# Harvard-AI-and-Robotics-Lab/FairFedMed

Measured on AMD Instinct MI355X. Metric: images/sec per client-round, ViT-B/16 FairLoRA r=8, bs=32 224^2, higher is better.
Workload: dtype bf16; 1 GPU; configs[1]: 1-client ViT-B/16 FairLoRA rank=8 G=3, bs=32 synthetic 224x224x3, fwd+bwd+SGD per step; global_batch=32, clients=1, trainable_elems=741952, loss_finite=1, launch=replay, rccl_ranks=1

## Files before the change

### fairfedmed_amd/_lib.py

```python
from __future__ import annotations

import ctypes as C
import os
from typing import Optional

import torch

_HERE = os.path.dirname(os.path.abspath(__file__))
LIB_PATH = os.environ.get("FFM_LIB_PATH") or os.path.join(_HERE, "csrc", "libffm_hip.so")

F32, BF16, F32_X3, F16 = 0, 1, 2, 3
F32_X3_W16 = 4
EPI_BIAS, EPI_LORA, EPI_LORA_KR, EPI_RESIDUAL, EPI_GELU, EPI_DGELU, EPI_RANKOP = 1, 2, 4, 8, 16, 32, 64
EPI_ROWSTATS, EPI_LNIN, EPI_LGRAD, EPI_BNBWD = 128, 256, 512, 1024
EPI_LNB_STAT, EPI_LNB_APPLY = 2048, 4096
EPI_GELU_ONLY = 8192
ABI_VERSION = 14
FILTERS = {"bilinear": 0, "bicubic": 1}

_vp, _i32, _i64, _f32 = C.c_void_p, C.c_int32, C.c_int64, C.c_float


class GemmArgs(C.Structure):
    _fields_ = [
# ... 79 lines not shown
    "ffm_ot_head_fwd": [_vp] * 10 + [_i32] * 6 + [_f32, _f32, _i32, _f32, _i32, _vp],
    "ffm_ot_head_bwd": [_vp] * 8 + [_i32] * 6 + [_vp],
    "ffm_expand_u8": [_vp, _vp, _i32, _i32, _i32, _i32, _vp],
    "ffm_resize_u8": [_vp, _vp, _vp, _vp, _vp, _i32, _i32, _i32, _i32, _i32, _vp],
    "ffm_augment_taps": [_i32, _i32, _i32],
    "ffm_augment_boxes": [_vp, _vp, _i32, _i64, _i32, _i32, _i32, _vp, _vp, _vp],
    "ffm_crop_resize_u8": [_vp, _vp, _vp, _vp, _i32, _i32, _i32, _i32, _i32, _i32, _vp],
    "ffm_scale_check": [_vp, _f32, _i64, _vp, _vp],
    "ffm_attention_fwd": [_vp, _vp, _vp, _i32, _i32, _i32, _i32, _i32, _vp],
    "ffm_attention_bwd": [_vp, _vp, _vp, _vp, _vp, _vp, _i32, _i32, _i32, _i32, _i32, _vp],
    "ffm_attention_bwd_lnstat_ok": [_i32, _i32, _i32],
    "ffm_attention_route": [_i32, _i32, _i32],
    "ffm_attention_bwd_lnstat": [_vp, _vp, _vp, _vp, _vp, _vp, _vp, _vp, _vp, _i32, _i32, _i32, _i32, _i32, _vp],
    "ffm_lora_down": [_vp, _i32, _vp, _i32, _vp, _vp, _i32, _i32, _i32, _i32, _i32, _f32, _f32, _vp, _vp, _vp, _vp,
                      _i32, _vp],
    "ffm_lora_down_blocks": [_i32, _i32, _i32, _i32],
    "ffm_lora_down_blocks_max": [_i32, _i32, _i32, _i32],
    "ffm_lora_grad_partial": [_vp, _i32, _vp, _i32, _i32, _i32, _vp, _i32, _vp],
    "ffm_lora_grad_partial_ln": [_vp, _i32, _vp, _vp, _vp, _vp, _vp, _i32, _i32, _i32, _vp, _i32, _vp],
    "ffm_lora_grad_splits": [_i32],
    "ffm_reduce_partials": [_vp, _i32, _i32, _vp, _i32, _i32, _i32, _vp],
    "ffm_reduce_partials_multi": [_vp, _i32, _i32, _vp],
    "ffm_head_fwd": [_vp, _vp, _vp, _vp, _vp, _vp, _i32, _i32, _i32, _i32, _i32, _vp],
    "ffm_ce_loss": [_vp, _vp, _vp, _vp, _vp, _vp, _vp, _i32, _i32, _i32, _vp],
    "ffm_ce_fair_loss": [_vp] * 10 + [_i32, _i32, _i32, _i32, _f32, _i32, _vp],
    "ffm_head_bwd": [_vp, _vp, _vp, _vp, _vp, _vp, _vp, _vp, _i32, _i32, _i32, _i32, _i32, _vp],
    "ffm_text_embed": [_vp, _vp, _vp, _i32, _vp, _vp, _i32, _i32, _i32, _i32, _i32, _vp],
    "ffm_text_tail_fwd": [_vp] * 10 + [_i32] * 4 + [_vp],
    "ffm_text_tail_bwd": [_vp] * 11 + [_i32] * 5 + [_vp],
    "ffm_text_ctx_grad": [_vp, _vp, _i32, _i32, _i32, _i32, _i32, _vp],
    "ffm_sgd_momentum": [_vp, _vp, _vp, _i64, _f32, _f32, _f32, _i32, _vp],
    "ffm_sgd_momentum_n": [_vp, _vp, _vp, _i64, _f32, _f32, _f32, _i32, _i32, _vp],
    "ffm_sgd_momentum_dev": [_vp, _vp, _vp, _i64, _vp, _i32, _vp, _vp],
    "ffm_loss_scale": [_vp, _i64, _vp, _vp],
    "ffm_unscale_check": [_vp, _i64, _vp, _vp],
    "ffm_sgd_momentum_gated": [_vp, _vp, _vp, _i64, _f32, _f32, _f32, _i32, _i32, _vp, _vp],
    "ffm_optim_state_rows": [_i32],
    "ffm_optim_step": [_vp, _vp, _vp, _i64, _i32, _vp, _i32, _vp, _vp],
    "ffm_optim_step_dev": [_vp, _vp, _vp, _i64, _i32, _vp, _i32, _vp, _vp],
    "ffm_scale_by": [_vp, _vp, _vp, _i64, _vp],
    "ffm_scale_acc": [_vp, _vp, _vp, _i64, _vp],
    "ffm_fedavg_finish": [_vp, _vp, _vp, _i64, _vp, _i32, _i32, _i32, _i32, _f32, _vp],
    "ffm_dp_norm_ws_bytes": [_i64],
    "ffm_dp_norm": [_vp, _vp, _i64, _vp, _vp],
    "ffm_dp_privatise": [_vp, _vp, _vp, _vp, _i64, _vp, _f32, _f32, _i64, _i32, _i32, _i32, _vp, _vp],
    "ffm_dp_noise": [_vp, _i64, _f32, _i64, _i32, _i32, _vp],
# ... 57 lines not shown
```

### fairfedmed_amd/csrc/head.hip

```cpp
#include "common.h"

namespace {

constexpr int HD_MAXV = 4;
constexpr int HD_MAXC = 8;

constexpr int HD_NW = 16;

template <typename T>
__global__ __launch_bounds__(64 * HD_NW) void head_fwd_kernel(const T* __restrict__ f, const float* __restrict__ tbar,
                                                       const float* __restrict__ logit_scale,
                                                       float* __restrict__ fbar, float* __restrict__ rnorm,
                                                       float* __restrict__ logits, int L, int D, int n_cls) {
    __shared__ float red[HD_NW / 2][4 * 64 * HD_MAXV];
    const int b = blockIdx.x, lane = threadIdx.x & 63, wave = threadIdx.x >> 6;
    const int nchunk = D >> 2;
    f32x4 acc[HD_MAXV];
#pragma unroll
    for (int i = 0; i < HD_MAXV; ++i) acc[i] = (f32x4){0.f, 0.f, 0.f, 0.f};
    for (int l = 1 + wave; l < L; l += HD_NW) {
        const T* fr = f + ((size_t)b * L + l) * D;
        f32x4 v[HD_MAXV];
        float ss = 0.f;
#pragma unroll
// ... 35 lines not shown
            if (c < nchunk) {
#pragma unroll
                for (int e = 0; e < 4; ++e) red[wave][c * 4 + e] += acc[i][e];
            }
        }
    }
    __syncthreads();
    const float inv = 1.0f / (float)(L - 1);
    for (int d = threadIdx.x; d < D; d += 64 * HD_NW) {
        float s = 0.f;
#pragma unroll
        for (int w = 0; w < HD_NW / 2; ++w) s += red[w][d];
        s *= inv;
        red[0][d] = s;
        fbar[(size_t)b * D + d] = s;
    }
    __syncthreads();
    const float scale = expf(logit_scale[0]);
    for (int c = wave; c < n_cls; c += HD_NW) {
        float s = 0.f;
        for (int d = lane; d < D; d += 64) s += red[0][d] * tbar[(size_t)c * D + d];
        s = wave_sum(s);
        if (lane == 0) logits[(size_t)b * n_cls + c] = scale * s;
    }
}

__global__ __launch_bounds__(256) void ce_loss_kernel(const float* __restrict__ logits_img,
                                                      const int64_t* __restrict__ label, float* __restrict__ logits,
                                                      float* __restrict__ prob, float* __restrict__ loss,
                                                      float* __restrict__ dlogits_img, int32_t* __restrict__ finite,
                                                      int nb, int S, int n_cls) {
    __shared__ float part[256];
    float my = 0.f;
    for (int b = threadIdx.x; b < nb; b += 256) {
        float lg[HD_MAXC];
        float mx = -INFINITY;
        for (int c = 0; c < n_cls; ++c) {
            float s = 0.f;
            for (int k = 0; k < S; ++k) s += logits_img[((size_t)b * S + k) * n_cls + c];
            lg[c] = s / (float)S;
            logits[(size_t)b * n_cls + c] = lg[c];
            mx = fmaxf(mx, lg[c]);
        }
        float se = 0.f;
        for (int c = 0; c < n_cls; ++c) se += expf(lg[c] - mx);
        const float lse = mx + logf(se);
// ... 209 lines not shown
            fb[u] = fbar[(size_t)(b + u) * D + d];
        }
#pragma unroll
        for (int u = 0; u < 8; ++u) s += dl[u] * fb[u];
    }
    for (; b < B; ++b) s += dlogits[(size_t)b * n_cls + c] * fbar[(size_t)b * D + d];
    dtbar[i] = s * expf(logit_scale[0]);
}

}

extern "C" int ffm_head_fwd(const void* f, const float* tbar, const float* logit_scale, float* fbar, float* rnorm,
                            float* logits_img, int B, int L, int D, int n_cls, int dtype, void* stream) {
    if (!f || !tbar || !logit_scale || !fbar || !rnorm || !logits_img) return FFM_EINVAL;
    if (B <= 0 || L <= 1 || D <= 0 || (D & 3) || D > 4 * 64 * HD_MAXV || n_cls <= 0 || n_cls > HD_MAXC) return FFM_EINVAL;
    hipStream_t s = (hipStream_t)stream;
    return ffm_by_storage(dtype, [&](auto tag) {
        typedef typename decltype(tag)::type T;
        hipLaunchKernelGGL((head_fwd_kernel<T>), dim3(B), dim3(64 * HD_NW), 0, s, (const T*)f, tbar, logit_scale, fbar, rnorm,
                           logits_img, L, D, n_cls);
        FFM_CHECK_LAUNCH();
        return FFM_OK;
    });
}

extern "C" int ffm_ce_loss(const float* logits_img, const int64_t* label, float* logits, float* prob, float* loss,
                           float* dlogits_img, int32_t* finite_flag, int nb, int S, int n_cls, void* stream) {
    if (!logits_img || !label || !logits || !prob || !loss || !dlogits_img) return FFM_EINVAL;
    if (nb <= 0 || S <= 0 || n_cls <= 0 || n_cls > HD_MAXC) return FFM_EINVAL;
    hipLaunchKernelGGL(ce_loss_kernel, dim3(1), dim3(256), 0, (hipStream_t)stream, logits_img, label, logits, prob,
                       loss, dlogits_img, finite_flag, nb, S, n_cls);
    FFM_CHECK_LAUNCH();
    return FFM_OK;
}

extern "C" int ffm_ce_fair_loss(const float* logits_img, const int64_t* label, const int32_t* attr, float* logits,
                                float* prob, float* loss, float* terms, float* gstat, float* dlogits_img,
                                int32_t* finite_flag, int nb, int S, int n_cls, int G, float lambda, int with_grad,
                                void* stream) {
    if (!logits_img || !label || !attr || !logits || !prob || !loss || !terms || !dlogits_img) return FFM_EINVAL;
    if (nb <= 0 || S <= 0 || n_cls <= 0 || n_cls > HD_MAXC || G <= 0 || G > FFM_MAX_GROUPS) return FFM_EINVAL;
    hipLaunchKernelGGL(ce_fair_loss_kernel, dim3(1), dim3(256), 0, (hipStream_t)stream, logits_img, label, attr, logits,
                       prob, loss, terms, gstat, dlogits_img, finite_flag, nb, S, n_cls, G, lambda, with_grad ? 1 : 0);
    FFM_CHECK_LAUNCH();
    return FFM_OK;
}
// ... 21 lines not shown
```

### fairfedmed_amd/csrc/lora.hip

```cpp
#include "common.h"

namespace {

constexpr int LD_WAVES = 8;
constexpr int LD_LDS_BUDGET = 64 * 1024;

template <int V>
__device__ __forceinline__ void reduce_scatter64(float (&vals)[V], int lane) {
#pragma unroll
    for (int n = V, o = 32; o >= 1; n >>= 1, o >>= 1) {
        const bool up = (lane & o) != 0;
#pragma unroll
        for (int i = 0; i < n / 2; ++i) {
            const float a = vals[i], b = vals[i + n / 2];
            const float keep = up ? b : a, send = up ? a : b;
            vals[i] = keep + __shfl_xor(send, o, 64);
        }
    }
}

template <typename T, int RP>
__global__ __launch_bounds__(LD_WAVES * 64) void lora_down_kernel(
    const T* __restrict__ x, int ldx, const float* __restrict__ P, int layout_rk, const float* __restrict__ S,
    const int32_t* __restrict__ attr, int M, int K, int r, int G, int rows_per_sample, float scaling,
// ... 120 lines not shown
        float sbv = 0.f;
        for (int g = 0; g < G; ++g) sbv += group_mix_w(attr, sample, g, G, lambda_group) * S[g * rs + j0 + oj];
        if (t_out) t_out[(size_t)orow * rs + j0 + oj] = tval;
        if (ts_out) ts_out[(size_t)orow * rs + j0 + oj] = scaling * tval * sbv;
    }
    if (t_fwd && ds_part) {
        if (kq == 0)
            Vs[(rg * RSUB + lane / RP) * RP + oj] = writer ? scaling * t_fwd[(size_t)orow * rs + j0 + oj] * tval : 0.f;
        __syncthreads();
        if (tid < G * r) {
            const int g = tid / r, j = tid % r;
            float s = 0.f;
            for (int rr = 0; rr < rows_blk; ++rr) {
                const int grow = blockIdx.x * rows_blk + rr;
                if (grow < M) s += group_mix_w(attr, grow / rows_per_sample, g, G, lambda_group) * Vs[rr * RP + j];
            }
            ds_part[((size_t)blockIdx.x * G + g) * rs + j0 + j] = s;
        }
    }
}

constexpr int LDM_ROWS = 16, LDM_WAVES = 4, LDM_U = 4;

__global__ __launch_bounds__(LDM_WAVES * 64) void lora_down_mfma_kernel(
    const bf16_t* __restrict__ x, int ldx, const float* __restrict__ P, const float* __restrict__ S,
    const int32_t* __restrict__ attr, int M, int K, int r, int G, int rows_per_sample, float scaling, float lambda_group,
    float* __restrict__ t_out, float* __restrict__ ts_out, const float* __restrict__ t_fwd, float* __restrict__ ds_part) {
    __shared__ f32x4 red[LDM_WAVES][64];
    __shared__ float dsum[(FFM_MAX_GROUPS + 2) * 16];
    const int tid = threadIdx.x, lane = tid & 63, wave = tid >> 6;
    const int col = lane & 15, kgp = lane >> 4;
    const int row0 = blockIdx.x * LDM_ROWS;
    int arow = row0 + col;
    arow = arow < M ? arow : M - 1;
    const int ksl = K / LDM_WAVES;
    const bf16_t* xa = x + (size_t)arow * ldx + wave * ksl + kgp * 8;
    const float* pb = P + (size_t)(col < r ? col : 0) * K + wave * ksl + kgp * 8;
    const bool bok = col < r;
    f32x4 acc = {0.f, 0.f, 0.f, 0.f};
    const int steps = ksl >> 5;
    for (int s0 = 0; s0 < steps; s0 += LDM_U) {
        bf16x8 av[LDM_U];
        f32x4 b0[LDM_U], b1[LDM_U];
#pragma unroll
        for (int u = 0; u < LDM_U; ++u) {
            const int st = s0 + u < steps ? s0 + u : steps - 1;
            av[u] = *reinterpret_cast<const bf16x8*>(xa + st * 32);
            b0[u] = *reinterpret_cast<const f32x4*>(pb + st * 32);
            b1[u] = *reinterpret_cast<const f32x4*>(pb + st * 32 + 4);
        }
#pragma unroll
        for (int u = 0; u < LDM_U; ++u) {
            if (s0 + u >= steps) break;
            bf16x8 bv;
#pragma unroll
            for (int e = 0; e < 4; ++e) {
                bv[e] = bok ? (bf16_t)b0[u][e] : (bf16_t)0.f;
                bv[4 + e] = bok ? (bf16_t)b1[u][e] : (bf16_t)0.f;
            }
            acc = __builtin_amdgcn_mfma_f32_16x16x32_bf16(bv, av[u], acc, 0, 0, 0);
        }
    }
    red[wave][lane] = acc;
    __syncthreads();
    if (wave != 0) return;
    f32x4 t4 = red[0][lane];
#pragma unroll
    for (int w = 1; w < LDM_WAVES; ++w) {
        const f32x4 o = red[w][lane];
#pragma unroll
        for (int e = 0; e < 4; ++e) t4[e] += o[e];
    }
    const int grow = row0 + col;
    const bool rok = grow < M;
    const int sample = (rok ? grow : M - 1) / rows_per_sample;
    const int ga = attr ? group_id(attr[sample], G) : -1;
    const float w_own = lambda_group, w_oth = (1.0f - lambda_group) / (float)(G > 1 ? G - 1 : 1), w_uni = 1.0f / (float)G;
    const bool do_ds = t_fwd && ds_part;
    float wv[4];
#pragma unroll
    for (int e = 0; e < 4; ++e) {
        const int j = 4 * kgp + e;
        wv[e] = 0.f;
        if (j < r && rok) {
            float sb = 0.f;
            for (int g = 0; g < G; ++g) sb += (ga < 0 ? w_uni : (ga == g ? w_own : w_oth)) * S[g * r + j];
            if (t_out) t_out[(size_t)grow * r + j] = t4[e];
            if (ts_out) ts_out[(size_t)grow * r + j] = scaling * t4[e] * sb;
            if (do_ds) wv[e] = scaling * t_fwd[(size_t)grow * r + j] * t4[e];
        }
    }
    if (!do_ds) return;
    float d_all[4], d_uni[4];
#pragma unroll
    for (int e = 0; e < 4; ++e) {
        d_all[e] = ga < 0 ? 0.f : wv[e];
        d_uni[e] = ga < 0 ? wv[e] : 0.f;
    }
    auto rows16 = [](float v) {
#pragma unroll
        for (int o = 1; o < 16; o <<= 1) v += __shfl_xor(v, o, 64);
        return v;
    };
#pragma unroll
    for (int e = 0; e < 4; ++e) {
        d_all[e] = rows16(d_all[e]);
        d_uni[e] = rows16(d_uni[e]);
    }
    if (col == 0) {
#pragma unroll
        for (int e = 0; e < 4; ++e) {
            dsum[0 * 16 + 4 * kgp + e] = d_all[e];
            dsum[1 * 16 + 4 * kgp + e] = d_uni[e];
        }
    }
    for (int g = 0; g < G; ++g) {
#pragma unroll
        for (int e = 0; e < 4; ++e) {
            const float o = rows16(ga == g ? wv[e] : 0.f);
            if (col == 0) dsum[(2 + g) * 16 + 4 * kgp + e] = o;
        }
    }
    __builtin_amdgcn_s_waitcnt(0xc07f);
    __builtin_amdgcn_wave_barrier();
    if (lane < G * r) {
        const int g = lane / r, j = lane % r;
        ds_part[((size_t)blockIdx.x * G + g) * r + j] = w_uni * dsum[16 + j] + w_oth * dsum[j] + (w_own - w_oth) * dsum[(2 + g) * 16 + j];
    }
    for (int i = lane + 64; i < G * r; i += 64) {
        const int g = i / r, j = i % r;
        ds_part[((size_t)blockIdx.x * G + g) * r + j] = w_uni * dsum[16 + j] + w_oth * dsum[j] + (w_own - w_oth) * dsum[(2 + g) * 16 + j];
    }
}

static bool down_mfma_ok(int M, int K, int r, int dtype, int layout_rk) {
    return dtype == FFM_BF16 && layout_rk && r <= 16 && M >= 1024 && K % (32 * LDM_WAVES) == 0;
}

static int down_kq(int K, int es) {
    const int nch = K * es / 16;
    return nch >= 256 ? 4 : nch >= 96 ? 2 : 1;
}
static int down_rp(int r, int dtype) { return r <= 4 && dtype == FFM_F32 ? 4 : r <= 8 ? 8 : 16; }

template <typename T, int RP>
int launch_down(const void* x, int ldx, const float* P, int layout_rk, const float* S, const int32_t* attr, int M,
                int K, int r, int G, int rps, float scaling, float lam, float* t, float* ts, const float* t_fwd,
                float* ds_part, int rs, int j0, hipStream_t s) {
    constexpr int CE = Elem<T>::kPerChunk;
    int ktile = K;
    const int per_col = RP * (int)sizeof(T);
    if (K * per_col > LD_LDS_BUDGET) ktile = (LD_LDS_BUDGET / per_col) / (64 * CE) * (64 * CE);
    const int lds = ktile * per_col;
    const int kq = down_kq(K, (int)sizeof(T));
    const int rows = (LD_WAVES / kq) * (64 / RP);
// ... 374 lines not shown
}
extern "C" int ffm_lora_down_blocks_max(int M_max, int K, int r, int dtype) {
    const int valu = down_valu_blocks(M_max, K, r, dtype);
    const int mf = down_mfma_ok(M_max, K, r, dtype, 1) ? (M_max + LDM_ROWS - 1) / LDM_ROWS : 0;
    return mf > valu ? mf : valu;
}
extern "C" int ffm_lora_grad_splits(int M) { return (M + LG_ROWS - 1) / LG_ROWS; }

extern "C" int ffm_lora_down(const void* x, int ldx, const float* P, int layout_rk, const float* S,
                             const int32_t* attr, int M, int K, int r, int G, int rows_per_sample, float scaling,
                             float lambda_group, float* t, float* ts, const float* t_fwd, float* ds_part, int dtype,
                             void* stream) {
    if (!x || !P || !S || M <= 0 || K <= 0 || r <= 0 || r > FFM_MAX_RANK || G <= 0 || G > FFM_MAX_GROUPS ||
        rows_per_sample <= 0)
        return FFM_EINVAL;
    if ((t_fwd == nullptr) != (ds_part == nullptr)) return FFM_EINVAL;
    if (G * r > 256) return FFM_EUNSUP;
    const size_t es = dtype == FFM_BF16 ? 2 : 4;
    if (dtype != FFM_BF16 && dtype != FFM_F32) return FFM_EINVAL;
    if (((size_t)K * es) % 16 || ((size_t)ldx * es) % 16 || ((uintptr_t)x & 15)) return FFM_EINVAL;
    if (ldx < K) return FFM_EINVAL;
    hipStream_t s = (hipStream_t)stream;
    if (down_mfma_ok(M, K, r, dtype, layout_rk)) {
        hipLaunchKernelGGL(lora_down_mfma_kernel, dim3((M + LDM_ROWS - 1) / LDM_ROWS), dim3(LDM_WAVES * 64), 0, s, (const bf16_t*)x,
                           ldx, P, S, attr, M, K, r, G, rows_per_sample, scaling, lambda_group, t, ts, t_fwd, ds_part);
        FFM_CHECK_LAUNCH();
        return FFM_OK;
    }
#define DOWN(RP, RR, J0) launch_down<T, RP>(x, ldx, P, layout_rk, S, attr, M, K, RR, G, rows_per_sample, scaling, \
                                            lambda_group, t, ts, t_fwd, ds_part, r, J0, s)
    return ffm_by_storage(dtype, [&](auto tag) {
        typedef typename decltype(tag)::type T;
        if (r > 16) {
            int e = DOWN(16, 16, 0);
            if (e) return e;
            return DOWN(16, r - 16, 16);
        }
        if constexpr (sizeof(T) == 4) {
            if (r <= 4) return DOWN(4, r, 0);
        }
        return r <= 8 ? DOWN(8, r, 0) : DOWN(16, r, 0);
    });
#undef DOWN
}

extern "C" int ffm_lora_grad_partial(const void* x, int ldx, const float* v, int M, int K, int r, float* part,
                                     int dtype, void* stream) {
    if (!x || !v || !part || M <= 0 || K <= 0 || r <= 0 || r > FFM_MAX_RANK) return FFM_EINVAL;
// ... 57 lines not shown
```

### fairfedmed_amd/engine.py

```python
from __future__ import annotations

import contextlib
import os
from dataclasses import dataclass
from typing import Dict, List, Optional, Tuple

import torch

from . import _lib as L
from ._lib import is16 as _is16
from . import ops
from .config import ModelCfg
from .data import NativeBatch
from .lora_site import LoraSite
from .synth import manifest, trainable_keys

Tensor = torch.Tensor


def _round_up(x: int, m: int) -> int:
    return (x + m - 1) // m * m


class FlatParams:
# ... 313 lines not shown


class _InferWorkspace:

    def __init__(self, eng: "FairLoRAEngine", max_images: int):
        cfg, v, dtype, dev = eng.cfg, eng.cfg.vision, eng.dtype, eng.device
        self.max_images = max_images
        T, w, P, r = max_images * v.tokens, v.width, v.grid * v.grid, cfg.lora.rank
        f32 = torch.float32
        e = lambda *s: torch.zeros(*s, device=dev, dtype=dtype)
        f = lambda *s: torch.zeros(*s, device=dev, dtype=f32)
        self.xs = (e(T, w), e(T, w))
        self.xm, self.qkv, self.o, self.h, self.h2, self.act = e(T, w), e(T, 3 * w), e(T, w), e(T, w), e(T, w), e(T, 4 * w)
        fold = _can_fold(r, dtype)
        self.rowps = (f(8 * T * 2), f(8 * T * 2)) if fold else None
        self.rowp2 = f(8 * T * 2) if fold else None
        self.t, self.ts = (f(T, r), f(T, r)) if (r and not eng.fused_rank) else (None, None)
        self.cols = e(max_images * P, 3 * v.patch * v.patch)
        self.patch_out = e(max_images * P, w)
        self.hpost = e(T, w)
        self.post_stats = (None, None)
        self.feat = e(T, v.out_dim)
        self.fbar = f(max_images, v.out_dim)
        self.rnorm = f(T)
        self.logits_img = f(max_images, cfg.n_cls)
        self.attr_i32 = torch.zeros(max_images, device=dev, dtype=torch.int32)
        if eng.is3d:
            H = v.image_size
            self.conv_out = f(max_images, 3, H, H)
            self.mm_part = f(max_images * ops.slice_blocks(H, H) * 2)
            self.mnmx = f(max_images, 2)
            self.mm_cnt = torch.zeros(max_images, 2, device=dev, dtype=torch.int32)
        if eng.ot:
            n = max_images * cfg.n_cls * (v.tokens - 1) * cfg.n_prompts
            self.ot_sim, self.ot_T = f(n), f(n)
            self.ot_errs = f(cfg.ot_max_iter * max_images * cfg.n_cls)
            self.ot_istop = torch.zeros(1, device=dev, dtype=torch.int32)
            self.ot_tsum = f(max_images * cfg.n_cls)

    def layer(self, i: int, rows: int) -> _LayerBufs:
        a, b = self.xs[i & 1], self.xs[(i + 1) & 1]
        rp, tts = self.rowps, (self.t, self.ts)
        return _LayerBufs(a[:rows], self.xm[:rows], self.qkv[:rows], self.o[:rows], self.h[:rows], self.h2[:rows], None,
                          self.act[:rows], b[:rows], rowp=rp[i & 1] if rp else None, rowp_out=rp[(i + 1) & 1] if rp else None,
                          rowp2=self.rowp2, in_proj=tts, out_proj=tts, c_fc=tts, c_proj=tts)

# ... 61 lines not shown
        self.sw = Switches.from_env()
        self.fused_rank = 0 < cfg.lora.rank <= 16
        self.pack_plan = None
        self._pack_event = None
        self.pk_out: Dict[str, Tensor] = {}
        self.use_replay = True
        self.params = FlatParams(cfg, self.device)
        self.params.load(state_dict)
        self.n_text = cfg.n_prompts * cfg.n_cls
        self.txt_len = min(t.context_length, max(cfg.eot) + 1)
        assert self.txt_len >= 1 + cfg.n_ctx
        if not all(0 <= int(e) < self.txt_len for e in cfg.eot):
            raise ValueError(f"EOT positions {list(cfg.eot)} must lie inside the {self.txt_len} text rows that are kept "
                             f"(context_length {t.context_length})")
        self.txt = _Stack(t.width, t.heads, t.layers, self.txt_len, self.n_text, True, 0, torch.float32, self.device,
                          self.sw, x3=(_is16(dtype)))
        dev, f32 = self.device, torch.float32
        self._init_vision(max_images)
        self.load_frozen(state_dict)
        self._init_vision_late()
        self.feat = torch.zeros(max_images * v.tokens, v.out_dim, device=dev, dtype=dtype)
        self.dfeat = torch.zeros_like(self.feat)
        self.fbar = torch.zeros(max_images, v.out_dim, device=dev, dtype=f32)
        self.rnorm = torch.zeros(max_images * v.tokens, device=dev, dtype=f32)
        self.logits_img = torch.zeros(max_images, cfg.n_cls, device=dev, dtype=f32)
        self.dlogits_img = torch.zeros_like(self.logits_img)
        self.logits = torch.zeros(max_images, cfg.n_cls, device=dev, dtype=f32)
        self.prob = torch.zeros_like(self.logits)
        self.loss = torch.zeros(1, device=dev, dtype=f32)
        self.finite = torch.ones(1, device=dev, dtype=torch.int32)
        self.scale_state = None
        if dtype == torch.float16:
            s0 = self.sw.f16_grad_scale
            self.scale_state = torch.tensor([s0, 1.0 / s0, 1.0, 0.0, 0.0, s0, self.sw.f16_growth_interval, 1.0],
                                            device=dev, dtype=f32)
        self.dtbar = torch.zeros(cfg.n_cls, v.out_dim, device=dev, dtype=f32)
        self.attr_i32 = torch.zeros(max_images, device=dev, dtype=torch.int32)
        self.label_buf = torch.zeros(max_images, device=dev, dtype=torch.int64)
        self._counts_buf = None
        self._fair_lam, self._fair_grad, self._fair_step = 0.0, False, False
        self.loss_terms = torch.zeros(2, device=dev, dtype=f32)
        self.group_conf = torch.zeros(ops.MAX_GROUPS, 2, device=dev, dtype=f32)
        self.tbar_buf = torch.zeros(cfg.n_cls, v.out_dim, device=dev, dtype=f32)
        self.ot = cfg.ot if cfg.ot != "None" else None
        if self.ot:
            if self.ot not in ops.OT_MODES:
# ... 371 lines not shown
            return ops.resize_u8(image, stage[:b])
        return ops.expand_u8(image.contiguous(), stage[:b], rep)

    def _pack_rank_operands(self) -> None:
        if self.pack_plan is not None:
            self.pack_plan.run()

    def _rank_operands_ready(self) -> None:
        ev = self._pack_event
        if ev is None:
            self._pack_rank_operands()
        else:
            self._ev_wait(torch.cuda.current_stream(self.device), ev)

    def _head_forward(self, rows: int, images: int, L: int, ws=None) -> None:
        cfg = self.cfg
        ws = self if ws is None else ws
        if self.ot:
            ops.ot_head_fwd(ws.feat[:rows], self.tn_buf, self.logit_scale, ws.rnorm, ws.ot_sim, ws.ot_T, ws.ot_errs,
                            ws.ot_istop, ws.ot_tsum, ws.logits_img, images, L, cfg.n_cls, cfg.n_prompts, self.ot,
                            cfg.ot_eps, cfg.ot_thresh, cfg.ot_max_iter, cfg.ot_top_percent)
        else:
            ops.head_fwd(ws.feat[:rows], self.tbar_buf, self.logit_scale, ws.fbar, ws.rnorm, ws.logits_img,
                         images, L, cfg.n_cls)

    def _head_backward(self, rows: int, images: int, L: int) -> None:
        cfg = self.cfg
        if self.ot:
            P = cfg.n_prompts * cfg.n_cls
            ops.ot_head_bwd(self.feat[:rows], self.tn_buf, self.logit_scale, self.rnorm, self.ot_T, self.dlogits_img,
                            self.dfeat[:rows], self.ot_dtn_part, images, L, cfg.n_cls, cfg.n_prompts)
            ops.reduce_partials(self.ot_dtn_part, images, P * self.cfg.vision.out_dim, self.dtn.view(-1))
        else:
            ops.head_bwd(self.feat[:rows], self.tbar_buf, self.logit_scale, self.fbar, self.rnorm, self.dlogits_img,
                         self.dfeat[:rows], self.dtbar, images, L, cfg.n_cls)

    @torch.no_grad()
    def forward(self, image: Tensor, attr: Optional[Tensor] = None) -> Tensor:
        if self.sops.type != "FairLoRA":
            attr = None
        b, S = self._load_inputs(image, attr, None)
        self._text_forward(False)
        self._vision_forward(b, S, attr is not None)
        return self.logits_img[:b * S].view(b, S, -1).mean(1)

    def _step_body(self, b: int, S: int, has_attr: bool) -> None:
        cfg, v = self.cfg, self.cfg.vision
# ... 430 lines not shown
```

### fairfedmed_amd/ops.py

```python
from __future__ import annotations

import ctypes as C
from typing import Optional

import torch

from . import _lib as L

Tensor = torch.Tensor

_REC = None


class record:
    def __init__(self, plan: list):
        self.plan = plan

    def __enter__(self):
        global _REC
        self.prev, _REC = _REC, self.plan
        return self.plan

    def __exit__(self, *a):
        global _REC
# ... 734 lines not shown
    M, K = x.shape
    if attr is not None:
        assert attr.dtype == torch.int32
    _call("ffm_lora_down", L.ptr(x), _ld(x), L.ptr(_f32(P)), int(layout_rk), L.ptr(_f32(S)), L.ptr(attr), M,
                                   K, r, G, rows_per_sample, scaling, lambda_group, L.ptr(_f32(t)), L.ptr(_f32(ts)),
                                   L.ptr(_f32(t_fwd)), L.ptr(_f32(ds_part)), L.dtype_code(x.dtype), L.stream_ptr())


def lora_grad_partial(x: Tensor, v: Tensor, r: int, part: Tensor) -> None:
    _dev(x, v, part)
    M, K = x.shape
    _call("ffm_lora_grad_partial", L.ptr(x), _ld(x), L.ptr(_f32(v)), M, K, r, L.ptr(_f32(part)),
                                           L.dtype_code(x.dtype), L.stream_ptr())


def reduce_partials(part: Tensor, nsplit: int, n: int, out: Tensor, transpose_K: int = 0, transpose_r: int = 0,
                    accumulate: bool = False) -> None:
    _dev(part, out)
    _call("ffm_reduce_partials", L.ptr(_f32(part)), nsplit, n, L.ptr(out), transpose_K, transpose_r,
                                         int(accumulate), L.stream_ptr())


def head_fwd(f: Tensor, tbar: Tensor, logit_scale: Tensor, fbar: Tensor, rnorm: Tensor, logits_img: Tensor, B: int,
             Ltok: int, n_cls: int) -> None:
    _dev(f, tbar, logit_scale, fbar, rnorm, logits_img)
    D = f.shape[1]
    assert f.is_contiguous()
    _call("ffm_head_fwd", L.ptr(f), L.ptr(_f32(tbar)), L.ptr(_f32(logit_scale)), L.ptr(_f32(fbar)),
                                  L.ptr(_f32(rnorm)), L.ptr(_f32(logits_img)), B, Ltok, D, n_cls,
                                  L.dtype_code(f.dtype), L.stream_ptr())


def text_embed(prefix: Tensor, ctx: Tensor, suffix: Tensor, pos: Tensor, x: Tensor, n_cls: int, TL: int) -> None:
    _dev(prefix, ctx, suffix, pos, x)
    n_prompts, n_ctx, w = ctx.shape
    for t in (prefix, ctx, suffix, pos, x):
        assert t.dtype == torch.float32 and t.is_contiguous()
    assert prefix.shape[0] == suffix.shape[0] == n_prompts * n_cls and x.shape[0] >= n_prompts * n_cls * TL and pos.shape[0] >= TL
    _call("ffm_text_embed", L.ptr(prefix), L.ptr(ctx), L.ptr(suffix), suffix.shape[1], L.ptr(pos), L.ptr(x), n_prompts, n_cls,
          n_ctx, TL, w, L.stream_ptr())


def text_tail_fwd(x: Tensor, eot_row: Tensor, lnw: Tensor, lnb: Tensor, proj: Tensor, tf: Tensor, tn: Tensor, rnorm: Tensor,
                  stats: Tensor, tbar: Optional[Tensor], n_prompts: int, n_cls: int) -> None:
    _dev(x, eot_row, lnw, lnb, proj, tf, tn, rnorm, stats, tbar)
    assert eot_row.dtype == torch.int32 and x.dtype == torch.float32 and proj.dtype == torch.float32 and proj.is_contiguous()
    w, D = proj.shape
    assert x.shape[1] == w and tf.shape == tn.shape == (n_prompts * n_cls, D) and tf.is_contiguous() and tn.is_contiguous()
    _call("ffm_text_tail_fwd", L.ptr(x), L.ptr(eot_row), L.ptr(lnw), L.ptr(lnb), L.ptr(proj), L.ptr(tf), L.ptr(tn), L.ptr(rnorm),
          L.ptr(stats), L.ptr(tbar), n_prompts, n_cls, w, D, L.stream_ptr())


def text_tail_bwd(x: Tensor, eot_row: Tensor, lnw: Tensor, proj: Tensor, tn: Tensor, rnorm: Tensor, stats: Tensor,
# ... 214 lines not shown
```

### include/ffm_hip.h

```cpp
#ifndef FFM_HIP_H
#define FFM_HIP_H

#include <stdint.h>

#ifdef __cplusplus
extern "C" {
#endif

#define FFM_F32 0
#define FFM_BF16 1
#define FFM_F32_X3 2
#define FFM_F16 3
#define FFM_F32_X3_W16 4

#define FFM_OK 0
#define FFM_EINVAL (-1)
#define FFM_EUNSUP (-2)

#define FFM_MAX_RANK 32
#define FFM_MAX_GROUPS 8

#define FFM_ABI_VERSION 14
int ffm_abi_version(void);

// ... 161 lines not shown
int ffm_lora_down_blocks_max(int M_max, int K, int r, int dtype);

int ffm_lora_grad_partial(const void* x, int ldx, const float* v, int M, int K, int r,
                          float* part, int dtype, void* stream);
int ffm_lora_grad_partial_ln(const void* x, int ldx, const float* v, const float* mean, const float* rstd,
                             const float* gamma, const float* beta, int M, int K, int r, float* part, int dtype,
                             void* stream);
int ffm_lora_grad_splits(int M);

int ffm_reduce_partials(const float* part, int nsplit, int n, float* out, int transpose_K,
                        int transpose_r, int accumulate, void* stream);

typedef struct ffm_reduce_desc {
    const float* part;
    float* out;
    int32_t nsplit, n, transpose_K, transpose_r;
} ffm_reduce_desc;
int ffm_reduce_partials_multi(const ffm_reduce_desc* descs_dev, int ndesc, int max_n, void* stream);

int ffm_head_fwd(const void* f, const float* tbar, const float* logit_scale, float* fbar,
                 float* rnorm, float* logits_img, int B, int L, int D, int n_cls, int dtype,
                 void* stream);

int ffm_ce_loss(const float* logits_img, const int64_t* label, float* logits, float* prob,
                float* loss, float* dlogits_img, int32_t* finite_flag, int nb, int S, int n_cls,
                void* stream);

int ffm_ce_fair_loss(const float* logits_img, const int64_t* label, const int32_t* attr,
                     float* logits, float* prob, float* loss, float* terms, float* gstat,
                     float* dlogits_img, int32_t* finite_flag, int nb, int S, int n_cls, int G,
                     float lambda, int with_grad, void* stream);

int ffm_head_bwd(const void* f, const float* tbar, const float* logit_scale, const float* fbar,
                 const float* rnorm, const float* dlogits_img, void* df, float* dtbar, int B,
                 int L, int D, int n_cls, int dtype, void* stream);

int ffm_text_embed(const float* prefix, const float* ctx, const float* suffix, int suffix_rows, const float* pos, float* x,
                   int n_prompts, int n_cls, int n_ctx, int TL, int w, void* stream);
int ffm_text_tail_fwd(const float* x, const int32_t* eot_row, const float* lnw, const float* lnb, const float* proj,
                      float* tf, float* tn, float* rnorm, float* stats, float* tbar, int n_prompts, int n_cls, int w,
                      int D, void* stream);
int ffm_text_tail_bwd(const float* x, const int32_t* eot_row, const float* lnw, const float* proj, const float* tn,
                      const float* rnorm, const float* stats, const float* dtbar, const float* dtn, float* dy, float* g,
                      int n_prompts, int n_cls, int TL, int w, int D, void* stream);
int ffm_text_ctx_grad(const float* g, float* dctx, int n_prompts, int n_cls, int n_ctx, int TL, int w, void* stream);

// ... 92 lines not shown
```

Baseline: 7031 images/sec.

## Split head forward over token slices and add async-LDS LoRA down kernel

```diff
diff --git a/fairfedmed_amd/_lib.py b/fairfedmed_amd/_lib.py
--- a/fairfedmed_amd/_lib.py
+++ b/fairfedmed_amd/_lib.py
@@ -125,6 +125,8 @@
     "ffm_reduce_partials": [_vp, _i32, _i32, _vp, _i32, _i32, _i32, _vp],
     "ffm_reduce_partials_multi": [_vp, _i32, _i32, _vp],
     "ffm_head_fwd": [_vp, _vp, _vp, _vp, _vp, _vp, _i32, _i32, _i32, _i32, _i32, _vp],
+    "ffm_head_fwd_slices": [],
+    "ffm_head_fwd_sliced": [_vp, _vp, _vp, _vp, _vp, _vp, _vp, _i32, _i32, _i32, _i32, _i32, _vp],
     "ffm_ce_loss": [_vp, _vp, _vp, _vp, _vp, _vp, _vp, _i32, _i32, _i32, _vp],
     "ffm_ce_fair_loss": [_vp] * 10 + [_i32, _i32, _i32, _i32, _f32, _i32, _vp],
     "ffm_head_bwd": [_vp, _vp, _vp, _vp, _vp, _vp, _vp, _vp, _i32, _i32, _i32, _i32, _i32, _vp],
diff --git a/fairfedmed_amd/csrc/head.hip b/fairfedmed_amd/csrc/head.hip
--- a/fairfedmed_amd/csrc/head.hip
+++ b/fairfedmed_amd/csrc/head.hip
@@ -81,6 +81,120 @@
         for (int d = lane; d < D; d += 64) s += red[0][d] * tbar[(size_t)c * D + d];
         s = wave_sum(s);
         if (lane == 0) logits[(size_t)b * n_cls + c] = scale * s;
+    }
+}
+
+constexpr int HD_NS = 8;
+constexpr int HD_SW = 8;
+constexpr int HD_RIF = 4;
+
+template <typename T, int NV>
+__global__ __launch_bounds__(64 * HD_SW) void head_slice_kernel(const T* __restrict__ f, float* __restrict__ part,
+                                                                float* __restrict__ rnorm, int L, int D) {
+    __shared__ f32x4 red[HD_SW][64 * NV];
+    const int b = blockIdx.x, s = blockIdx.y, lane = threadIdx.x & 63, wave = threadIdx.x >> 6;
+    const int nchunk = D >> 2;
+    const int per = (L - 1 + HD_NS - 1) / HD_NS;
+    const int l0 = 1 + s * per, l1 = min(L, l0 + per);
+    int col[NV];
+    bool live[NV];
+#pragma unroll
+    for (int i = 0; i < NV; ++i) {
+        const int c = lane + 64 * i;
+        live[i] = c < nchunk;
+        col[i] = (live[i] ? c : nchunk - 1) * 4;
+    }
+    f32x4 acc[NV];
+#pragma unroll
+    for (int i = 0; i < NV; ++i) acc[i] = (f32x4){0.f, 0.f, 0.f, 0.f};
+    for (int lb = l0 + wave; lb < l1; lb += HD_SW * HD_RIF) {
+        f32x4 v[HD_RIF][NV];
+#pragma unroll
+        for (int u = 0; u < HD_RIF; ++u) {
+            const int l = min(lb + u * HD_SW, l1 - 1);
+            const T* fr = f + ((size_t)b * L + l) * D;
+#pragma unroll
+            for (int i = 0; i < NV; ++i) v[u][i] = Vec4<T>::load(fr + col[i]);
+        }
+#pragma unroll
+        for (int u = 0; u < HD_RIF; ++u) {
+            const int l = lb + u * HD_SW;
+            float ss = 0.f;
+#pragma unroll
+            for (int i = 0; i < NV; ++i) {
+                const float q = v[u][i][0] * v[u][i][0] + v[u][i][1] * v[u][i][1] + v[u][i][2] * v[u][i][2] +
+                                v[u][i][3] * v[u][i][3];
+                ss += live[i] ? q : 0.f;
+            }
+            const float rn = 1.0f / fmaxf(sqrtf(wave_sum(ss)), 1e-12f);
+            if (l < l1) {
+                if (lane == 0) rnorm[(size_t)b * L + l] = rn;
+#pragma unroll
+                for (int i = 0; i < NV; ++i) {
+#pragma unroll
+                    for (int e = 0; e < 4; ++e) acc[i][e] += v[u][i][e] * rn;
+                }
+            }
+        }
+    }
+    if (s == 0 && threadIdx.x == 0) rnorm[(size_t)b * L] = 0.f;
+#pragma unroll
+    for (int i = 0; i < NV; ++i) red[wave][lane + 64 * i] = acc[i];
+    __syncthreads();
+    float* pr = part + ((size_t)b * HD_NS + s) * D;
+    for (int c = threadIdx.x; c < nchunk; c += 64 * HD_SW) {
+        f32x4 t = red[0][c];
+#pragma unroll
+        for (int w = 1; w < HD_SW; ++w) t += red[w][c];
+        *reinterpret_cast<f32x4*>(pr + c * 4) = t;
+    }
+}
+
+__global__ __launch_bounds__(256) void head_finish_kernel(const float* __restrict__ part, const float* __restrict__ tbar,
+                                                          const float* __restrict__ logit_scale,
+                                                          float* __restrict__ fbar, float* __restrict__ logits, int L,
+                                                          int D, int n_cls) {
+    __shared__ float fb[4 * 64 * HD_MAXV];
+    const int b = blockIdx.x, lane = threadIdx.x & 63, wave = threadIdx.x >> 6;
+    const int c = threadIdx.x;
+    constexpr int NT = 4 * HD_MAXV;
+    const float ls = logit_scale[0];
+    float tv[2][NT];
+#pragma unroll
+    for (int q = 0; q < 2; ++q) {
+        const int k = wave + 4 * q;
+        const float* tr = tbar + (size_t)(k < n_cls ? k : 0) * D;
+#pragma unroll
+        for (int i = 0; i < NT; ++i) {
+            const int d = lane + 64 * i;
+            tv[q][i] = tr[d < D ? d : 0];
+        }
+    }
+    if (c < (D >> 2)) {
+        const float* pr = part + (size_t)b * HD_NS * D + c * 4;
+        f32x4 p[HD_NS];
+#pragma unroll
+        for (int s = 0; s < HD_NS; ++s) p[s] = *reinterpret_cast<const f32x4*>(pr + (size_t)s * D);
+        f32x4 t = p[0];
+#pragma unroll
+        for (int s = 1; s < HD_NS; ++s) t += p[s];
+        t *= 1.0f / (float)(L - 1);
+        *reinterpret_cast<f32x4*>(fb + c * 4) = t;
+        *reinterpret_cast<f32x4*>(fbar + (size_t)b * D + c * 4) = t;
+    }
+    __syncthreads();
+    const float scale = expf(ls);
+#pragma unroll
+    for (int q = 0; q < 2; ++q) {
+        const int k = wave + 4 * q;
+        float s = 0.f;
+#pragma unroll
+        for (int i = 0; i < NT; ++i) {
+            const int d = lane + 64 * i;
+            s += d < D ? fb[d] * tv[q][i] : 0.f;
+        }
+        s = wave_sum(s);
+        if (lane == 0 && k < n_cls) logits[(size_t)b * n_cls + k] = scale * s;
     }
 }
 
@@ -336,6 +450,32 @@
         FFM_CHECK_LAUNCH();
         return FFM_OK;
     });
+}
+
+extern "C" int ffm_head_fwd_slices(void) { return HD_NS; }
+
+extern "C" int ffm_head_fwd_sliced(const void* f, const float* tbar, const float* logit_scale, float* fbar, float* rnorm,
+                                   float* logits_img, float* ws, int B, int L, int D, int n_cls, int dtype, void* stream) {
+    if (!f || !tbar || !logit_scale || !fbar || !rnorm || !logits_img || !ws) return FFM_EINVAL;
+    if (B <= 0 || L <= 1 || D <= 0 || (D & 3) || D > 4 * 64 * HD_MAXV || n_cls <= 0 || n_cls > HD_MAXC)
+        return FFM_EINVAL;
+    hipStream_t s = (hipStream_t)stream;
+    const int e = ffm_by_storage(dtype, [&](auto tag) {
+        typedef typename decltype(tag)::type T;
+        const dim3 grid(B, HD_NS), block(64 * HD_SW);
+        switch ((D + 255) / 256) {
+            case 1: hipLaunchKernelGGL((head_slice_kernel<T, 1>), grid, block, 0, s, (const T*)f, ws, rnorm, L, D); break;
+            case 2: hipLaunchKernelGGL((head_slice_kernel<T, 2>), grid, block, 0, s, (const T*)f, ws, rnorm, L, D); break;
+            case 3: hipLaunchKernelGGL((head_slice_kernel<T, 3>), grid, block, 0, s, (const T*)f, ws, rnorm, L, D); break;
+            default: hipLaunchKernelGGL((head_slice_kernel<T, 4>), grid, block, 0, s, (const T*)f, ws, rnorm, L, D); break;
+        }
+        FFM_CHECK_LAUNCH();
+        return FFM_OK;
+    });
+    if (e != FFM_OK) return e;
+    hipLaunchKernelGGL(head_finish_kernel, dim3(B), dim3(256), 0, s, ws, tbar, logit_scale, fbar, logits_img, L, D, n_cls);
+    FFM_CHECK_LAUNCH();
+    return FFM_OK;
 }
 
 extern "C" int ffm_ce_loss(const float* logits_img, const int64_t* label, float* logits, float* prob, float* loss,
diff --git a/fairfedmed_amd/csrc/lora.hip b/fairfedmed_amd/csrc/lora.hip
--- a/fairfedmed_amd/csrc/lora.hip
+++ b/fairfedmed_amd/csrc/lora.hip
@@ -166,6 +166,106 @@
 
 constexpr int LDM_ROWS = 16, LDM_WAVES = 4, LDM_U = 4;
 
+struct down_row {
+    int ga;
+    float sb[4], tf[4];
+};
+__device__ __forceinline__ down_row down_mfma_row(int lane, int row0, const float* __restrict__ S,
+                                                  const int32_t* __restrict__ attr, int M, int r, int G, int rows_per_sample,
+                                                  float lambda_group, const float* __restrict__ t_fwd) {
+    const int col = lane & 15, kgp = lane >> 4;
+    const int grow = row0 + col;
+    const bool rok = grow < M;
+    const int sample = (rok ? grow : M - 1) / rows_per_sample;
+    down_row rc;
+    rc.ga = attr ? group_id(attr[sample], G) : -1;
+    const float w_own = lambda_group, w_oth = (1.0f - lambda_group) / (float)(G > 1 ? G - 1 : 1), w_uni = 1.0f / (float)G;
+#pragma unroll
+    for (int e = 0; e < 4; ++e) {
+        const int j = 4 * kgp + e;
+        rc.sb[e] = 0.f;
+        rc.tf[e] = 0.f;
+        if (j < r && rok) {
+            float sb = 0.f;
+            for (int g = 0; g < G; ++g) sb += (rc.ga < 0 ? w_uni : (rc.ga == g ? w_own : w_oth)) * S[g * r + j];
+            rc.sb[e] = sb;
+            if (t_fwd) rc.tf[e] = t_fwd[(size_t)grow * r + j];
+        }
+    }
+    return rc;
+}
+
+__device__ __forceinline__ void down_mfma_finish(f32x4 (&red)[LDM_WAVES][64], float (&dsum)[(FFM_MAX_GROUPS + 2) * 16],
+                                                 const down_row& rc, int lane, int row0, int M, int r, int G, float scaling,
+                                                 float lambda_group, float* __restrict__ t_out, float* __restrict__ ts_out,
+                                                 const float* __restrict__ t_fwd, float* __restrict__ ds_part) {
+    const int col = lane & 15, kgp = lane >> 4;
+    f32x4 t4 = red[0][lane];
+#pragma unroll
+    for (int w = 1; w < LDM_WAVES; ++w) {
+        const f32x4 o = red[w][lane];
+#pragma unroll
+        for (int e = 0; e < 4; ++e) t4[e] += o[e];
+    }
+    const int grow = row0 + col;
+    const bool rok = grow < M;
+    const int ga = rc.ga;
+    const float w_own = lambda_group, w_oth = (1.0f - lambda_group) / (float)(G > 1 ? G - 1 : 1), w_uni = 1.0f / (float)G;
+    const bool do_ds = t_fwd && ds_part;
+    float wv[4];
+#pragma unroll
+    for (int e = 0; e < 4; ++e) {
+        const int j = 4 * kgp + e;
+        wv[e] = 0.f;
+        if (j < r && rok) {
+            if (t_out) t_out[(size_t)grow * r + j] = t4[e];
+            if (ts_out) ts_out[(size_t)grow * r + j] = scaling * t4[e] * rc.sb[e];
+            if (do_ds) wv[e] = scaling * rc.tf[e] * t4[e];
+        }
+    }
+    if (!do_ds) return;
+    float d_all[4], d_uni[4];
+#pragma unroll
+    for (int e = 0; e < 4; ++e) {
+        d_all[e] = ga < 0 ? 0.f : wv[e];
+        d_uni[e] = ga < 0 ? wv[e] : 0.f;
+    }
+    auto rows16 = [](float v) {
+#pragma unroll
+        for (int o = 1; o < 16; o <<= 1) v += __shfl_xor(v, o, 64);
+        return v;
+    };
+#pragma unroll
+    for (int e = 0; e < 4; ++e) {
+        d_all[e] = rows16(d_all[e]);
+        d_uni[e] = rows16(d_uni[e]);
+    }
+    if (col == 0) {
+#pragma unroll
+        for (int e = 0; e < 4; ++e) {
+            dsum[0 * 16 + 4 * kgp + e] = d_all[e];
+            dsum[1 * 16 + 4 * kgp + e] = d_uni[e];
+        }
+    }
+    for (int g = 0; g < G; ++g) {
+#pragma unroll
+        for (int e = 0; e < 4; ++e) {
+            const float o = rows16(ga == g ? wv[e] : 0.f);
+            if (col == 0) dsum[(2 + g) * 16 + 4 * kgp + e] = o;
+        }
+    }
+    __builtin_amdgcn_s_waitcnt(0xc07f);
+    __builtin_amdgcn_wave_barrier();
+    if (lane < G * r) {
+        const int g = lane / r, j = lane % r;
+        ds_part[((size_t)blockIdx.x * G + g) * r + j] = w_uni * dsum[16 + j] + w_oth * dsum[j] + (w_own - w_oth) * dsum[(2 + g) * 16 + j];
+    }
+    for (int i = lane + 64; i < G * r; i += 64) {
+        const int g = i / r, j = i % r;
+        ds_part[((size_t)blockIdx.x * G + g) * r + j] = w_uni * dsum[16 + j] + w_oth * dsum[j] + (w_own - w_oth) * dsum[(2 + g) * 16 + j];
+    }
+}
+
 __global__ __launch_bounds__(LDM_WAVES * 64) void lora_down_mfma_kernel(
     const bf16_t* __restrict__ x, int ldx, const float* __restrict__ P, const float* __restrict__ S,
     const int32_t* __restrict__ attr, int M, int K, int r, int G, int rows_per_sample, float scaling, float lambda_group,
@@ -181,6 +281,8 @@
     const bf16_t* xa = x + (size_t)arow * ldx + wave * ksl + kgp * 8;
     const float* pb = P + (size_t)(col < r ? col : 0) * K + wave * ksl + kgp * 8;
     const bool bok = col < r;
+    down_row rc = {};
+    if (wave == 0) rc = down_mfma_row(lane, row0, S, attr, M, r, G, rows_per_sample, lambda_group, t_fwd);
     f32x4 acc = {0.f, 0.f, 0.f, 0.f};
     const int steps = ksl >> 5;
     for (int s0 = 0; s0 < steps; s0 += LDM_U) {
@@ -208,73 +310,82 @@
     red[wave][lane] = acc;
     __syncthreads();
     if (wave != 0) return;
-    f32x4 t4 = red[0][lane];
-#pragma unroll
-    for (int w = 1; w < LDM_WAVES; ++w) {
-        const f32x4 o = red[w][lane];
-#pragma unroll
-        for (int e = 0; e < 4; ++e) t4[e] += o[e];
-    }
-    const int grow = row0 + col;
-    const bool rok = grow < M;
-    const int sample = (rok ? grow : M - 1) / rows_per_sample;
-    const int ga = attr ? group_id(attr[sample], G) : -1;
-    const float w_own = lambda_group, w_oth = (1.0f - lambda_group) / (float)(G > 1 ? G - 1 : 1), w_uni = 1.0f / (float)G;
-    const bool do_ds = t_fwd && ds_part;
-    float wv[4];
-#pragma unroll
-    for (int e = 0; e < 4; ++e) {
-        const int j = 4 * kgp + e;
-        wv[e] = 0.f;
-        if (j < r && rok) {
-            float sb = 0.f;
-            for (int g = 0; g < G; ++g) sb += (ga < 0 ? w_uni : (ga == g ? w_own : w_oth)) * S[g * r + j];
-            if (t_out) t_out[(size_t)grow * r + j] = t4[e];
-            if (ts_out) ts_out[(size_t)grow * r + j] = scaling * t4[e] * sb;
-            if (do_ds) wv[e] = scaling * t_fwd[(size_t)grow * r + j] * t4[e];
-        }
-    }
-    if (!do_ds) return;
-    float d_all[4], d_uni[4];
-#pragma unroll
-    for (int e = 0; e < 4; ++e) {
-        d_all[e] = ga < 0 ? 0.f : wv[e];
-        d_uni[e] = ga < 0 ? wv[e] : 0.f;
-    }
-    auto rows16 = [](float v) {
-#pragma unroll
-        for (int o = 1; o < 16; o <<= 1) v += __shfl_xor(v, o, 64);
-        return v;
+    down_mfma_finish(red, dsum, rc, lane, row0, M, r, G, scaling, lambda_group, t_out, ts_out, t_fwd, ds_part);
+}
+
+constexpr int LDX_TS = 2;
+constexpr int LDX_TILE = LDM_ROWS * 256;
+
+__global__ __launch_bounds__(LDM_WAVES * 64, 2) void lora_down_dma_kernel(
+    const bf16_t* __restrict__ x, int ldx, const float* __restrict__ P, const float* __restrict__ S,
+    const int32_t* __restrict__ attr, int M, int K, int r, int G, int rows_per_sample, float scaling, float lambda_group,
+    float* __restrict__ t_out, float* __restrict__ ts_out, const float* __restrict__ t_fwd, float* __restrict__ ds_part) {
+    __shared__ __attribute__((aligned(16))) char xs[LDM_WAVES * LDX_TS * LDX_TILE];
+    __shared__ f32x4 red[LDM_WAVES][64];
+    __shared__ float dsum[(FFM_MAX_GROUPS + 2) * 16];
+    const int tid = threadIdx.x, lane = tid & 63, wave = __builtin_amdgcn_readfirstlane(tid >> 6);
+    const int col = lane & 15, kgp = lane >> 4;
+    const int row0 = blockIdx.x * LDM_ROWS;
+    const int ksl = K / LDM_WAVES, steps = ksl >> 5, tiles = ksl >> 7;
+    const bf16_t* src[4];
+#pragma unroll
+    for (int q = 0; q < 4; ++q) {
+        const int rw = 4 * q + kgp;
+        int gr = row0 + rw;
+        gr = gr < M ? gr : M - 1;
+        src[q] = x + (size_t)gr * ldx + wave * ksl + ((col ^ rw) << 3);
+    }
+    char* mine = xs + wave * (LDX_TS * LDX_TILE);
+    const float* pb = P + (size_t)(col < r ? col : 0) * K + wave * ksl + kgp * 8;
+    const bool bok = col < r;
+    f32x4 b0[LDX_TS * 4], b1[LDX_TS * 4];
+    auto request = [&](int t0) {
+#pragma unroll
+        for (int t = 0; t < LDX_TS; ++t) {
+            if (t0 + t < tiles) {
+#pragma unroll
+                for (int q = 0; q < 4; ++q)
+                    __builtin_amdgcn_global_load_lds((const __attribute__((address_space(1))) void*)(src[q] + (t0 + t) * 128),
+                                                     (__attribute__((address_space(3))) void*)(mine + t * LDX_TILE + q * 1024),
+                                                     16, 0, 0);
+            }
+        }
+#pragma unroll
+        for (int i = 0; i < LDX_TS * 4; ++i) {
+            const int st = 4 * t0 + i < steps ? 4 * t0 + i : steps - 1;
+            b0[i] = *reinterpret_cast<const f32x4*>(pb + st * 32);
+            b1[i] = *reinterpret_cast<const f32x4*>(pb + st * 32 + 4);
+        }
     };
-#pragma unroll
-    for (int e = 0; e < 4; ++e) {
-        d_all[e] = rows16(d_all[e]);
-        d_uni[e] = rows16(d_uni[e]);
-    }
-    if (col == 0) {
-#pragma unroll
-        for (int e = 0; e < 4; ++e) {
-            dsum[0 * 16 + 4 * kgp + e] = d_all[e];
-            dsum[1 * 16 + 4 * kgp + e] = d_uni[e];
-        }
-    }
-    for (int g = 0; g < G; ++g) {
-#pragma unroll
-        for (int e = 0; e < 4; ++e) {
-            const float o = rows16(ga == g ? wv[e] : 0.f);
-            if (col == 0) dsum[(2 + g) * 16 + 4 * kgp + e] = o;
-        }
-    }
-    __builtin_amdgcn_s_waitcnt(0xc07f);
-    __builtin_amdgcn_wave_barrier();
-    if (lane < G * r) {
-        const int g = lane / r, j = lane % r;
-        ds_part[((size_t)blockIdx.x * G + g) * r + j] = w_uni * dsum[16 + j] + w_oth * dsum[j] + (w_own - w_oth) * dsum[(2 + g) * 16 + j];
-    }
-    for (int i = lane + 64; i < G * r; i += 64) {
-        const int g = i / r, j = i % r;
-        ds_part[((size_t)blockIdx.x * G + g) * r + j] = w_uni * dsum[16 + j] + w_oth * dsum[j] + (w_own - w_oth) * dsum[(2 + g) * 16 + j];
-    }
+    f32x4 acc = {0.f, 0.f, 0.f, 0.f};
+    request(0);
+    down_row rc = {};
+    if (wave == 0) rc = down_mfma_row(lane, row0, S, attr, M, r, G, rows_per_sample, lambda_group, t_fwd);
+    for (int t0 = 0; t0 < tiles; t0 += LDX_TS) {
+        asm volatile("s_waitcnt vmcnt(0)" ::: "memory");
+        bf16x8 av[LDX_TS * 4], bv[LDX_TS * 4];
+#pragma unroll
+        for (int i = 0; i < LDX_TS * 4; ++i) {
+            const int ch = 4 * (i & 3) + kgp;
+            av[i] = *reinterpret_cast<const bf16x8*>(mine + (i >> 2) * LDX_TILE + col * 256 + ((ch ^ col) << 4));
+#pragma unroll
+            for (int e = 0; e < 4; ++e) {
+                bv[i][e] = bok ? (bf16_t)b0[i][e] : (bf16_t)0.f;
+                bv[i][4 + e] = bok ? (bf16_t)b1[i][e] : (bf16_t)0.f;
+            }
+        }
+        asm volatile("s_waitcnt lgkmcnt(0)" ::: "memory");
+        if (t0 + LDX_TS < tiles) request(t0 + LDX_TS);
+#pragma unroll
+        for (int i = 0; i < LDX_TS * 4; ++i) {
+            if (4 * t0 + i >= steps) break;
+            acc = __builtin_amdgcn_mfma_f32_16x16x32_bf16(bv[i], av[i], acc, 0, 0, 0);
+        }
+    }
+    red[wave][lane] = acc;
+    __syncthreads();
+    if (wave != 0) return;
+    down_mfma_finish(red, dsum, rc, lane, row0, M, r, G, scaling, lambda_group, t_out, ts_out, t_fwd, ds_part);
 }
 
 static bool down_mfma_ok(int M, int K, int r, int dtype, int layout_rk) {
@@ -695,8 +806,13 @@
     if (ldx < K) return FFM_EINVAL;
     hipStream_t s = (hipStream_t)stream;
     if (down_mfma_ok(M, K, r, dtype, layout_rk)) {
-        hipLaunchKernelGGL(lora_down_mfma_kernel, dim3((M + LDM_ROWS - 1) / LDM_ROWS), dim3(LDM_WAVES * 64), 0, s, (const bf16_t*)x,
-                           ldx, P, S, attr, M, K, r, G, rows_per_sample, scaling, lambda_group, t, ts, t_fwd, ds_part);
+        const dim3 grid((M + LDM_ROWS - 1) / LDM_ROWS), block(LDM_WAVES * 64);
+        if (K % (128 * LDM_WAVES) == 0)
+            hipLaunchKernelGGL(lora_down_dma_kernel, grid, block, 0, s, (const bf16_t*)x, ldx, P, S, attr, M, K, r, G,
+                               rows_per_sample, scaling, lambda_group, t, ts, t_fwd, ds_part);
+        else
+            hipLaunchKernelGGL(lora_down_mfma_kernel, grid, block, 0, s, (const bf16_t*)x, ldx, P, S, attr, M, K, r, G,
+                               rows_per_sample, scaling, lambda_group, t, ts, t_fwd, ds_part);
         FFM_CHECK_LAUNCH();
         return FFM_OK;
     }
diff --git a/fairfedmed_amd/engine.py b/fairfedmed_amd/engine.py
--- a/fairfedmed_amd/engine.py
+++ b/fairfedmed_amd/engine.py
@@ -359,6 +359,7 @@
         self.post_stats = (None, None)
         self.feat = e(T, v.out_dim)
         self.fbar = f(max_images, v.out_dim)
+        self.head_ws = f(ops.head_fwd_ws_floats(max_images, v.out_dim))
         self.rnorm = f(T)
         self.logits_img = f(max_images, cfg.n_cls)
         self.attr_i32 = torch.zeros(max_images, device=dev, dtype=torch.int32)
@@ -466,6 +467,7 @@
         self.feat = torch.zeros(max_images * v.tokens, v.out_dim, device=dev, dtype=dtype)
         self.dfeat = torch.zeros_like(self.feat)
         self.fbar = torch.zeros(max_images, v.out_dim, device=dev, dtype=f32)
+        self.head_ws = torch.zeros(ops.head_fwd_ws_floats(max_images, v.out_dim), device=dev, dtype=f32)
         self.rnorm = torch.zeros(max_images * v.tokens, device=dev, dtype=f32)
         self.logits_img = torch.zeros(max_images, cfg.n_cls, device=dev, dtype=f32)
         self.dlogits_img = torch.zeros_like(self.logits_img)
@@ -883,7 +885,7 @@
                             cfg.ot_eps, cfg.ot_thresh, cfg.ot_max_iter, cfg.ot_top_percent)
         else:
             ops.head_fwd(ws.feat[:rows], self.tbar_buf, self.logit_scale, ws.fbar, ws.rnorm, ws.logits_img,
-                         images, L, cfg.n_cls)
+                         images, L, cfg.n_cls, ws.head_ws)
 
     def _head_backward(self, rows: int, images: int, L: int) -> None:
         cfg = self.cfg
diff --git a/fairfedmed_amd/ops.py b/fairfedmed_amd/ops.py
--- a/fairfedmed_amd/ops.py
+++ b/fairfedmed_amd/ops.py
@@ -780,13 +780,20 @@
 
 
 def head_fwd(f: Tensor, tbar: Tensor, logit_scale: Tensor, fbar: Tensor, rnorm: Tensor, logits_img: Tensor, B: int,
-             Ltok: int, n_cls: int) -> None:
-    _dev(f, tbar, logit_scale, fbar, rnorm, logits_img)
+             Ltok: int, n_cls: int, ws: Optional[Tensor] = None) -> None:
+    _dev(f, tbar, logit_scale, fbar, rnorm, logits_img, ws)
     D = f.shape[1]
     assert f.is_contiguous()
-    _call("ffm_head_fwd", L.ptr(f), L.ptr(_f32(tbar)), L.ptr(_f32(logit_scale)), L.ptr(_f32(fbar)),
-                                  L.ptr(_f32(rnorm)), L.ptr(_f32(logits_img)), B, Ltok, D, n_cls,
-                                  L.dtype_code(f.dtype), L.stream_ptr())
+    if ws is None:
+        ws = torch.empty(head_fwd_ws_floats(B, D), device=f.device, dtype=torch.float32)
+    assert ws.numel() >= head_fwd_ws_floats(B, D)
+    _call("ffm_head_fwd_sliced", L.ptr(f), L.ptr(_f32(tbar)), L.ptr(_f32(logit_scale)), L.ptr(_f32(fbar)),
+                                         L.ptr(_f32(rnorm)), L.ptr(_f32(logits_img)), L.ptr(_f32(ws)), B, Ltok, D, n_cls,
+                                         L.dtype_code(f.dtype), L.stream_ptr())
+
+
+def head_fwd_ws_floats(B: int, D: int) -> int:
+    return B * L.load().ffm_head_fwd_slices() * D
 
 
 def text_embed(prefix: Tensor, ctx: Tensor, suffix: Tensor, pos: Tensor, x: Tensor, n_cls: int, TL: int) -> None:
diff --git a/include/ffm_hip.h b/include/ffm_hip.h
--- a/include/ffm_hip.h
+++ b/include/ffm_hip.h
@@ -207,6 +207,11 @@
                  float* rnorm, float* logits_img, int B, int L, int D, int n_cls, int dtype,
                  void* stream);
 
+int ffm_head_fwd_slices(void);
+int ffm_head_fwd_sliced(const void* f, const float* tbar, const float* logit_scale, float* fbar,
+                        float* rnorm, float* logits_img, float* ws, int B, int L, int D, int n_cls,
+                        int dtype, void* stream);
+
 int ffm_ce_loss(const float* logits_img, const int64_t* label, float* logits, float* prob,
                 float* loss, float* dlogits_img, int32_t* finite_flag, int nb, int S, int n_cls,
                 void* stream);
```

Measured after the change: 7024 images/sec. Within noise of the previous version (-0.1%).
